# mrvollger/rustybam

Measured on NVIDIA B200. Metric: lifted window-records/s, higher is better.
Workload: dtype u32/u64 (+f32 identities)

## Files before the change

### rustybam_b200/csrc/rb_kernels.cu

```cuda
#include <algorithm>
#include <cstdio>

#include "f32_fmt.cuh"
#include "lift_core.cuh"
#include "rb_kernels.cuh"
#include "rec_core.cuh"
#include "stream_core.cuh"

namespace rb {

__device__ __forceinline__ uint4 ld_nc_v4(const void* p) {
    uint4 r;
    asm volatile("ld.global.nc.L1::no_allocate.v4.u32 {%0,%1,%2,%3}, [%4];" : "=r"(r.x), "=r"(r.y), "=r"(r.z), "=r"(r.w) : "l"(p));
    return r;
}
__device__ __forceinline__ unsigned long long ld_volatile_u64(const unsigned long long* p) {
    unsigned long long v;
    asm volatile("ld.volatile.global.u64 %0, [%1];" : "=l"(v) : "l"(p));
    return v;
}
__device__ __forceinline__ uint32_t ld_volatile_u32(const uint32_t* p) {
    uint32_t v;
    asm volatile("ld.volatile.global.u32 %0, [%1];" : "=r"(v) : "l"(p));
    return v;
// ... 712 lines not shown
        auto emit_e = [&](uint64_t p, const HalfE& hh) { store_half(&la.he[p], &hh); };
        if (staged) {
            SegRec s2 = sr;
            s2.s_lo = js0; s2.s_hi = js1; s2.e_lo = je0; s2.e_hi = je1;
            const WinStaged ws{s_ps, s_pe, js0, je0};
            stream_segment(v, s2, ws, first, (uint32_t)nvalid, seg_op, pre.c, mine.c.T, acc, emit_s, emit_e);
        } else {
            sr.s_lo = sr.e_lo = sr.wlo; sr.s_hi = sr.e_hi = sr.whi;
            stream_segment(v, sr, wg, first, (uint32_t)nvalid, seg_op, pre.c, mine.c.T, acc, emit_s, emit_e);
        }
        return;
    }

    if (nvalid == 0) return;
    const uint32_t hex = hpre + (hinc - hc);
    uint32_t r = r_blk + hex + ((tid > 0) ? (h & 1u) : 0u);
    int jb = 0;
    Ctr base = pre.c;
    for (;;) {
        const uint32_t hm = (jb >= 31) ? 0u : (h & ~((2u << jb) - 1u));
        const int je = hm ? (__ffs(hm) - 1) : nvalid;
        const uint64_t k0 = first + (uint64_t)jb;
        if (r < la.n_rec && la.op_off[r] <= k0 && k0 < la.op_off[r + 1]) {
            const RecInfo& R = la.recs[r];
            SegRec sr;
            sr.eo0 = R.eo0; sr.eo1 = R.eo1; sr.wlo = R.wlo; sr.whi = R.whi;
            sr.s_lo = sr.e_lo = sr.wlo; sr.s_hi = sr.e_hi = sr.whi;
            if (sr.whi > sr.wlo) {
                sr.pair0 = la.pair_off[la.rec_rank[r]];
                const WinGlobal wg{la.w_st, la.w_en, R.t_st, R.t_en};
                uint32_t Tseg = 0;
                for (int j = jb; j < je; j++) {
                    const uint32_t w = my_ops[j];
                    if (is_ref(op_code(w))) Tseg += op_len(w);
                }
                stream_segment(v, sr, wg, k0, (uint32_t)(je - jb), [&](uint32_t j) { return my_ops[jb + (int)j]; }, base, Tseg, acc,
                               [&](uint64_t p, const HalfS& hh) { store_half(&la.hs[p], &hh); },
                               [&](uint64_t p, const HalfE& hh) { store_half(&la.he[p], &hh); });
            }
        }
        if (je >= nvalid) break;
        jb = je;
        r++;
        base = ctr_zero();
    }
}

#ifndef RB_SMP2_MINB
#define RB_SMP2_MINB 4
#endif
#ifndef RB_SMP2_MINB_NOSUBS
#define RB_SMP2_MINB_NOSUBS 5
#endif
template <bool LOCAL, bool NOSUBS = false>
__global__ void __launch_bounds__(SMP_THREADS, NOSUBS ? RB_SMP2_MINB_NOSUBS : RB_SMP2_MINB)
k_samples2(const uint32_t* __restrict__ ops, const uint64_t* __restrict__ n_ops_dev, const uint32_t* __restrict__ heads,
           Ctr* __restrict__ samples, uint32_t* blk_state, ScanPayload* blk_agg, ScanPayload* blk_pre, unsigned int* ticket,
           uint32_t no_subs_arg ) {
    const bool no_subs = NOSUBS || no_subs_arg != 0u;
    static_assert(SAMPLE == 32u, "k_samples2 walks 32-op chunks");
    extern __shared__ __align__(16) uint32_t s_dyn2[];
    uint4* s_ops4 = reinterpret_cast<uint4*>(s_dyn2);
    uint32_t* s_acc = s_dyn2 + SMP_THREADS * SAMPLE;
    __shared__ SegVal s_warp[SMP_THREADS / 32];
    __shared__ SegVal s_blk;
    __shared__ unsigned int s_b;
    const int tid = threadIdx.x, lane = tid & 31, warp = tid >> 5;
    const uint64_t n_ops = *n_ops_dev;
    if (!LOCAL) {
        if (tid == 0) s_b = atomicAdd(ticket, 1u);
        __syncthreads();
    }
    const uint64_t b = LOCAL ? (uint64_t)blockIdx.x : (uint64_t)s_b;
    const uint64_t op0 = b * (uint64_t)SMP_OPS;
    if (op0 >= n_ops && !(n_ops == 0 && b == 0)) {
        if (LOCAL && tid == 0) payload_store(&blk_agg[b], seg_identity());
        return;
    }

    {
        const uint4* src = reinterpret_cast<const uint4*>(ops + op0);
#pragma unroll
        for (int i = 0; i < (int)SAMPLE / 4; i++) {
            const uint32_t v4 = (uint32_t)i * SMP_THREADS + tid;
            uint4 x = make_uint4(0u, 0u, 0u, 0u);
            if (op0 + (uint64_t)v4 * 4u < n_ops) x = src[v4];
            const uint32_t row = v4 >> 3, u = v4 & 7u;
            s_ops4[row * 8u + (u ^ (row & 7u))] = x;
        }
    }
    __syncthreads();

    const uint64_t chunk = b * SMP_THREADS + tid;
    const uint64_t first = chunk << SAMPLE_LOG2;
    int nvalid = 0;
    if (first < n_ops) nvalid = (n_ops - first) < SAMPLE ? (int)(n_ops - first) : (int)SAMPLE;
    const uint32_t h = nvalid ? heads[first >> 5] : 0u;
    const uint32_t sw = (uint32_t)tid & 7u;
    const uint4* row = s_ops4 + (uint32_t)tid * 8u;
    auto op_at = [&](int j) { return reinterpret_cast<const uint32_t*>(&row[((uint32_t)j >> 2) ^ sw])[j & 3]; };
    uint32_t prev_code = 99u;
    if (nvalid) {
        if (tid > 0) prev_code = op_code(s_ops4[(uint32_t)(tid - 1) * 8u + (7u ^ ((uint32_t)(tid - 1) & 7u))].w);
        else if (first > 0) prev_code = op_code(ops[first - 1]);
    }
    SegVal mine = seg_identity();
    ClassAcc acc;
    acc.sum = s_acc + tid; acc.stride = SMP_THREADS;
    acc_reset(acc);
    uint32_t slowc = 0;
    auto store_sub = [&](const Ctr& sub, uint32_t k) {
        uint4* dst = reinterpret_cast<uint4*>(samples + chunk * SUBS + k);
        const uint32_t* w = reinterpret_cast<const uint32_t*>(&sub);
        dst[0] = make_uint4(w[0], w[1], w[2], w[3]);
        dst[1] = make_uint4(w[4], w[5], w[6], w[7]);
        dst[2] = make_uint4(w[8], w[9], w[10], w[11]);
    };
    if (nvalid == (int)SAMPLE && h == 0u) {
        uint32_t iev = 0, dev = 0, txt = 0, big = 0;
#pragma unroll
        for (int u = 0; u < 8; u++) {
            if (u && !(u & 1) && !no_subs) {
                Ctr sub = ctr_zero();
                acc.iev = iev; acc.dev = dev; acc.txt = txt; acc.big = big;
                if (big >= ACC_BIG) { for (int t = 0; t < 4 * u; t++) ctr_add_op(sub, op_at(t)); }
                else acc_flush(acc, sub);
                sub.aux = 0u;
                store_sub(sub, (uint32_t)u >> 1);
            }
            const uint4 x = row[(uint32_t)u ^ sw];
            const uint32_t ws[4] = {x.x, x.y, x.z, x.w};
#pragma unroll
            for (int k = 0; k < 4; k++) {
                const uint32_t w = ws[k], code = op_code(w), n = op_len(w);
                acc.sum[code * SMP_THREADS] += n;
                iev += (code == OP_I);
                dev += (code == OP_D);
                txt += ndigits32(n) + 1u;
                big |= n;
                slowc += ((n - 1u) >= (ACC_BIG - 1u)) | (code == prev_code);
                prev_code = code;
            }
        }
        acc.iev = iev; acc.dev = dev; acc.txt = txt; acc.big = big;
        if (big >= ACC_BIG) { for (int j = 0; j < (int)SAMPLE; j++) ctr_add_op(mine.c, op_at(j)); }
        else acc_flush(acc, mine.c);
    } else {
        for (int j = 0; j < nvalid; j++) {
            const uint32_t w = op_at(j);
            const bool head = (h >> j) & 1u;
            if (head) { acc_reset(acc); slowc = 0; }
            if (j && (j & (int)(SUB_OPS - 1)) == 0 && !no_subs) {
                Ctr sub = ctr_zero();
                if (acc.big >= ACC_BIG) {
                    int j0 = 0;
                    for (int t = 0; t <= j; t++)
                        if ((h >> t) & 1u) j0 = t;
                    for (int t = j0; t < j; t++) ctr_add_op(sub, op_at(t));
                } else {
                    acc_flush(acc, sub);
                }
                sub.aux = (((h >> 1) & ((1u << j) - 1u)) != 0u) ? SUB_ABS : 0u;
                store_sub(sub, (uint32_t)(j >> SUB_LOG2));
            }
            const uint32_t code = op_code(w);
            slowc += (op_len(w) == 0u) | (op_len(w) >= ACC_BIG) | ((!head) & (code == prev_code));
            acc_add_op(acc, w);
            prev_code = code;
        }
        if (acc.big >= ACC_BIG) {
            int j0 = 0;
            for (int j = 0; j < nvalid; j++)
                if ((h >> j) & 1u) j0 = j;
            for (int j = j0; j < nvalid; j++) ctr_add_op(mine.c, op_at(j));
        } else {
            acc_flush(acc, mine.c);
        }
    }
    mine.c.aux = (mine.c.aux & AUX_OVF) | (slowc & AUX_CNT);
    mine.flag = (h != 0u);

    SegVal inc = mine;
#pragma unroll
    for (int d = 1; d < 32; d <<= 1) {
        const SegVal y = seg_shfl(inc, (lane - d) & 31);
        if (lane >= d) inc = seg_combine(y, inc);
    }
    if (lane == 31) s_warp[warp] = inc;
    SegVal exl = seg_shfl(inc, (lane - 1) & 31);
    if (lane == 0) exl = seg_identity();
    __syncthreads();
    SegVal wpre = seg_identity(), btot = seg_identity();
    if (LOCAL) {
        for (int k = 0; k < warp; k++) wpre = seg_combine(wpre, s_warp[k]);
        if (tid == SMP_THREADS - 1) payload_store(&blk_agg[b], seg_combine(wpre, inc));
        SegVal pre = seg_combine(wpre, exl);
        if (h & 1u) { pre.c = ctr_zero(); pre.flag = 1u; }
        if (nvalid) {
            pre.c.aux = (pre.c.aux & ~SUB_ABS) | (pre.flag ? SUB_ABS : 0u);
            samples[chunk * SUBS] = pre.c;
        }
        return;
    }
    if (warp == 0) {
#pragma unroll
        for (int k = 0; k < SMP_THREADS / 32; k++) btot = seg_combine(btot, s_warp[k]);
#if RB_SMP2_LB2
        const SegVal ex = lookback_seg2(blk_agg, b, btot);
#else
        const SegVal ex = lookback_seg(blk_state, blk_agg, blk_pre, b, btot);
#endif
        if (lane == 0) s_blk = ex;
    } else {
        for (int k = 0; k < warp; k++) wpre = seg_combine(wpre, s_warp[k]);
    }
    __syncthreads();
    SegVal pre = seg_combine(seg_combine(s_blk, wpre), exl);
    if (h & 1u) pre.c = ctr_zero();
    if (no_subs) pre.c.aux = (pre.c.aux & ~SUB_ABS) | SUB_ABS;
    if (nvalid) samples[chunk * SUBS] = pre.c;
}

constexpr uint32_t TS_NONE = 0xFFFFFFFFu;
__global__ void __launch_bounds__(256)
k_rec_heads(const uint8_t* __restrict__ text, const uint64_t* __restrict__ cigar_off, uint32_t n_rec, uint64_t* __restrict__ head_pos,
            uint32_t* tile_first) {
    const uint32_t r = blockIdx.x * blockDim.x + threadIdx.x;
    if (r >= n_rec) return;
    const uint64_t c = cigar_off[r], e = cigar_off[r + 1];
    uint64_t hp = ~0ull;
    const uint64_t lim = (e - c > 16u) ? c + 16u : e;
    for (uint64_t p = c; p < lim; p++)
        if (((uint32_t)text[p] - 48u) >= 10u) { hp = p; break; }
    head_pos[r] = hp;
    if (hp != ~0ull) atomicMin(&tile_first[hp / TOK_TILE], r);
}

#ifndef RB_TOKSCAN_MINB
#define RB_TOKSCAN_MINB 4
#endif
__global__ void __launch_bounds__(TOK_THREADS, RB_TOKSCAN_MINB)
k_tok_scan(const uint8_t* __restrict__ text, uint32_t* __restrict__ ops, unsigned long long* tile_state, unsigned int* ticket,
           ErrSlots err, uint32_t* misc_flags, const uint32_t* __restrict__ tile_first, const uint64_t* __restrict__ head_pos,
           uint32_t n_rec, Ctr* __restrict__ samples, uint32_t* seg_state, ScanPayload* seg_agg, ScanPayload* seg_pre) {
    __shared__ __align__(16) uint8_t s_text[16 + TOK_TILE + 16];
    __shared__ uint16_t s_pos[TOK_TILE / 2];
    __shared__ uint32_t s_opw[TOK_TILE / 2];
    __shared__ uint32_t s_head[TOK_TILE / 64 + 1];
    __shared__ uint16_t s_excl[TOK_THREADS], s_m16[TOK_THREADS];
    __shared__ uint8_t s_lut[256];
    __shared__ __align__(8) unsigned long long s_bar;
    __shared__ uint32_t s_warp[TOK_THREADS / 32];
    __shared__ SegVal s_wagg[TOK_THREADS / 32];
    __shared__ SegVal s_blk;
    __shared__ unsigned long long s_base;
    __shared__ unsigned int s_tile;
    __shared__ uint32_t s_prev0;

    const int tid = threadIdx.x, lane = tid & 31, warp = tid >> 5;
    if (tid < 256) s_lut[tid] = (uint8_t)code_of_char((uint32_t)tid);
    if (tid < TOK_TILE / 64 + 1) s_head[tid] = 0u;
    if (tid == 0) {
        s_tile = atomicAdd(ticket, 1u);
        mbar_init(&s_bar, 1);
        s_prev0 = 99u;
    }
    __syncthreads();
    const uint64_t tile = s_tile;
    const uint64_t tbase = tile * (uint64_t)TOK_TILE;
    if (tid == 0) {
        mbar_expect_tx(&s_bar, 16 + TOK_TILE);
        bulk_g2s(s_text, text + tbase - 16, 16 + TOK_TILE, &s_bar);
    }
// ... 1826 lines not shown
    const uint64_t c = (uint64_t)blockIdx.x * (WT_THREADS / 32) + warp;
    const uint64_t n_ops = op_off[n_rec];
    const uint64_t k0 = c << SAMPLE_LOG2;
    if (k0 >= n_ops) return;
    const uint64_t k1 = (k0 + SAMPLE < n_ops) ? k0 + SAMPLE : n_ops;
    const uint64_t k = k0 + lane;
    auto rec_of = [&](uint64_t op) {
        uint32_t lo = 0, hi = n_rec;
        while (lo < hi) {
            const uint32_t mid = lo + ((hi - lo) >> 1);
            if (op_off[mid] <= op) lo = mid + 1; else hi = mid;
        }
        return lo - 1;
    };
    auto body_of = [&](uint32_t r) { return line_off[r + 1] - 1 - recs[r].tot.TXT; };
    const uint32_t r0 = rec_of(k0);
    uint32_t w = 0, nb = 0;
    if (k < k1) { w = ops[k]; nb = ndigits32(op_len(w)) + 1u; }
    if (op_off[r0 + 1] >= k1) {
        uint32_t inc = nb;
#pragma unroll
        for (int d = 1; d < 32; d <<= 1) {
            const uint32_t t = __shfl_up_sync(0xffffffffu, inc, d);
            if (lane >= d) inc += t;
        }
        const uint32_t tot = __shfl_sync(0xffffffffu, inc, 31);
        const uint32_t base = (k0 > op_off[r0]) ? samples[c * SUBS].TXT : 0u;
        if (nb) put_op(&s_stage[warp][inc - nb], op_len(w), op_code(w));
        __syncwarp();
        uint8_t* dst = out_text + body_of(r0) + base;
        for (uint32_t i = lane; i < tot; i += 32) dst[i] = s_stage[warp][i];
        return;
    }
    if (k >= k1) return;
    const uint32_t r = rec_of(k);
    const uint64_t a = op_off[r];
    uint64_t j = a;
    uint32_t pos = 0;
    if (k0 > a) { j = k0; pos = samples[c * SUBS].TXT; }
    for (; j < k; j++) pos += ndigits32(op_len(ops[j])) + 1u;
    put_op(out_text + body_of(r) + pos, op_len(w), op_code(w));
}

static size_t samples2_smem() { return (size_t)(SMP_THREADS * SAMPLE + 9 * SMP_THREADS) * sizeof(uint32_t); }
static size_t scan_lift_smem(bool lift) {
    return (size_t)(SMP_THREADS * (SAMPLE + 1) + 9 * SMP_THREADS + (lift ? 2 * SL_WCAP : 0)) * sizeof(uint32_t);
}
int init_kernel_attrs() {
    cudaError_t e = cudaFuncSetAttribute(k_scan_lift<true>, cudaFuncAttributeMaxDynamicSharedMemorySize, (int)scan_lift_smem(true));
    if (e == cudaSuccess) e = cudaFuncSetAttribute(k_scan_lift<false>, cudaFuncAttributeMaxDynamicSharedMemorySize, (int)scan_lift_smem(false));
    if (e == cudaSuccess) e = cudaFuncSetAttribute(k_samples2<true>, cudaFuncAttributeMaxDynamicSharedMemorySize, (int)samples2_smem());
    if (e == cudaSuccess) e = cudaFuncSetAttribute(k_samples2<false>, cudaFuncAttributeMaxDynamicSharedMemorySize, (int)samples2_smem());
    if (e == cudaSuccess) e = cudaFuncSetAttribute(k_samples2<false, true>, cudaFuncAttributeMaxDynamicSharedMemorySize, (int)samples2_smem());
    if (e == cudaSuccess) e = cudaFuncSetAttribute(k_serialise, cudaFuncAttributeMaxDynamicSharedMemorySize, SER_CAP);
    if (e == cudaSuccess) e = cudaFuncSetAttribute(k_emit<false>, cudaFuncAttributeMaxDynamicSharedMemorySize, EMIT_DYN_BYTES);
    if (e == cudaSuccess) e = cudaFuncSetAttribute(k_emit<true>, cudaFuncAttributeMaxDynamicSharedMemorySize, EMIT_DYN_BYTES);
    return e == cudaSuccess ? 0 : -1;
}
__global__ void k_add_u64(unsigned long long* __restrict__ p, uint64_t n, unsigned long long delta) {
    const uint64_t i = (uint64_t)blockIdx.x * blockDim.x + threadIdx.x;
    if (i < n) p[i] += delta;
}
void launch_add_u64(uint64_t* p, uint64_t n, uint64_t delta, cudaStream_t s) {
    if (n == 0 || delta == 0) return;
    k_add_u64<<<(unsigned)((n + 255) / 256), 256, 0, s>>>(reinterpret_cast<unsigned long long*>(p), n, delta);
}
void launch_whole_text(const uint32_t* ops, const uint64_t* op_off, uint32_t n_rec, const RecInfo* recs, const Ctr* samples,
                       const uint64_t* line_off, uint8_t* out_text, uint64_t n_ops_bound, cudaStream_t s) {
    if (n_rec == 0 || n_ops_bound == 0 || out_text == nullptr) return;
    const uint64_t chunks = (n_ops_bound + SAMPLE - 1) / SAMPLE;
    k_whole_text<<<(unsigned)((chunks + WT_THREADS / 32 - 1) / (WT_THREADS / 32)), WT_THREADS, 0, s>>>(ops, op_off, n_rec, recs, samples,
                                                                                                    line_off, out_text);
}
void launch_tokenise(const uint8_t* text, uint64_t n_tiles, uint32_t* ops, unsigned long long* tile_state, unsigned int* ticket,
                     ErrSlots err, uint32_t* misc_flags, cudaStream_t s) {
    if (n_tiles == 0) return;
    k_tokenise<<<(unsigned)n_tiles, TOK_THREADS, 0, s>>>(text, ops, tile_state, ticket, err, misc_flags);
}
void launch_tok_scan(const uint8_t* text, uint64_t n_tiles, const uint64_t* cigar_off, uint32_t n_rec, uint32_t* ops,
                     unsigned long long* tile_state, unsigned int* ticket, ErrSlots err, uint32_t* misc_flags, uint32_t* tile_first,
                     uint64_t* head_pos, Ctr* samples, uint32_t* seg_state, ScanPayload* seg_agg, ScanPayload* seg_pre, cudaStream_t s) {
    if (n_tiles == 0) return;
    if (n_rec) k_rec_heads<<<(n_rec + 255) / 256, 256, 0, s>>>(text, cigar_off, n_rec, head_pos, tile_first);
    k_tok_scan<<<(unsigned)n_tiles, TOK_THREADS, 0, s>>>(text, ops, tile_state, ticket, err, misc_flags, tile_first, head_pos, n_rec,
                                                         samples, seg_state, seg_agg, seg_pre);
}
void launch_rec_ops(const uint8_t* text, const uint64_t* cigar_off, uint32_t n_rec, const unsigned long long* tile_state,
                    uint64_t* op_off, uint32_t* heads, ErrSlots err, cudaStream_t s) {
    const uint64_t warps = (uint64_t)n_rec + 1;
    k_rec_ops<<<(unsigned)((warps * 32 + 255) / 256), 256, 0, s>>>(text, cigar_off, n_rec, tile_state, op_off, heads, err);
}
void launch_scan_lift(bool lift, const uint32_t* ops, const uint64_t* n_ops_dev, uint64_t n_ops_bound, const uint32_t* heads,
                      Ctr* samples, uint32_t* blk_state, ScanPayload* blk_agg, ScanPayload* blk_pre, unsigned int* ticket,
                      LiftArgs la, cudaStream_t s, bool no_subs) {
    const uint64_t blocks = (n_ops_bound + SMP_OPS - 1) / SMP_OPS;
    if (blocks == 0) return;
    if (lift)
        k_scan_lift<true><<<(unsigned)blocks, SMP_THREADS, scan_lift_smem(true), s>>>(ops, n_ops_dev, heads, samples, blk_state, blk_agg,
                                                                                      blk_pre, ticket, la);
    else if (getenv("RB_OLD_SAMPLES"))
        k_scan_lift<false><<<(unsigned)blocks, SMP_THREADS, scan_lift_smem(false), s>>>(ops, n_ops_dev, heads, samples, blk_state,
                                                                                        blk_agg, blk_pre, ticket, la);
    else if (!getenv("RB_SAMPLES_LOCAL")) {
#if RB_SMP2_LB2
        cudaMemsetAsync(blk_agg, 0, blocks * sizeof(ScanPayload), s);
#endif
        if (no_subs)
            k_samples2<false, true><<<(unsigned)blocks, SMP_THREADS, samples2_smem(), s>>>(ops, n_ops_dev, heads, samples, blk_state, blk_agg, blk_pre,
                                                                                           ticket, 1u);
        else
            k_samples2<false><<<(unsigned)blocks, SMP_THREADS, samples2_smem(), s>>>(ops, n_ops_dev, heads, samples, blk_state, blk_agg, blk_pre, ticket,
                                                                                     0u);
    } else {
        k_samples2<true><<<(unsigned)blocks, SMP_THREADS, samples2_smem(), s>>>(ops, n_ops_dev, heads, samples, blk_state, blk_agg, blk_pre, ticket, 0u);
        k_blk_scan<<<1, 1024, 0, s>>>(n_ops_dev, blk_agg, blk_pre);
        const uint64_t chunks = (n_ops_bound + SAMPLE - 1) / SAMPLE;
        k_smp_fix<<<(unsigned)((chunks + 255) / 256), 256, 0, s>>>(n_ops_dev, blk_pre, samples);
    }
}
void launch_combine(uint64_t n_pairs, const uint64_t* pair_off, const uint32_t* rec_order, uint32_t n_rec, const RecInfo* recs,
                    const uint32_t* ops, WinView win, const uint64_t* names_off, const HalfS* hs, const HalfE* he, PairRes* res,
                    uint32_t* line_len, ErrSlots err, cudaStream_t s) {
    if (n_pairs == 0) return;
    k_combine<<<(unsigned)((n_pairs + 127) / 128), 128, 0, s>>>(n_pairs, pair_off, rec_order, n_rec, recs, ops, win, names_off, hs, he,
                                                                res, line_len, err);
}
void launch_check_clips(const uint32_t* ops, const uint64_t* op_off, uint32_t n_rec, ErrSlots err, cudaStream_t s) {
    if (n_rec == 0) return;
    k_check_clips<<<(n_rec + 127) / 128, 128, 0, s>>>(ops, op_off, n_rec, err);
}
void launch_rec_prep(int mode, RecInput in, const uint64_t* op_off, const uint32_t* ops, const Ctr* samples, WinView win,
                     RecInfo* recs, uint32_t* pair_cnt, StatsDev st, ErrSlots err, cudaStream_t s) {
    if (in.n_rec == 0) return;
    k_rec_prep<<<(in.n_rec + 127) / 128, 128, 0, s>>>(mode, in, op_off, ops, samples, win, recs, pair_cnt, st, err);
}
void launch_whole_rows(uint32_t n_rec, const RecInfo* recs, PairRes* res, uint32_t* line_len, uint64_t* pair_off, LiftPlan* plans,
                       cudaStream_t s) {
    k_whole_rows<<<n_rec / 128 + 1, 128, 0, s>>>(n_rec, recs, res, line_len, pair_off, plans);
}
void launch_pair_scan(const uint32_t* pair_cnt, const uint32_t* rec_order, uint32_t n_rec, uint64_t* pair_off, cudaStream_t s) {
    k_pair_scan<<<1, 1024, 0, s>>>(pair_cnt, rec_order, n_rec, pair_off);
}
void launch_lift_plan(uint64_t n_pairs, const uint64_t* pair_off, const uint32_t* rec_order, uint32_t n_rec, const RecInfo* recs,
                      const Ctr* samples, WinView win, LiftPlan* plans, cudaStream_t s, bool mark_fast) {
    if (n_pairs == 0) return;
    const uint32_t nb = (uint32_t)((n_pairs + LIFT_THREADS - 1) / LIFT_THREADS);
    k_lift_plan<<<(nb + 127) / 128, 128, 0, s>>>(n_pairs, nb, pair_off, rec_order, n_rec, recs, samples, win, plans, mark_fast ? 1u : 0u);
}
void launch_lift(uint64_t n_pairs, const uint64_t* pair_off, const uint32_t* rec_order, uint32_t n_rec, const RecInfo* recs,
                 const uint32_t* ops, const Ctr* samples, WinView win, const uint64_t* names_off, int policy, const LiftPlan* plans,
                 PairRes* res, uint32_t* line_len, ErrSlots err, cudaStream_t s, bool skip_fast, bool wide) {
    if (n_pairs == 0) return;
    const unsigned grid = (unsigned)((n_pairs + LIFT_THREADS - 1) / LIFT_THREADS);
    if (wide)
        k_lift<false><<<grid, LIFT_THREADS, 0, s>>>(n_pairs, pair_off, rec_order, n_rec, recs, ops, samples, win, names_off, policy, plans, res,
                                                    line_len, err, skip_fast ? 1u : 0u);
    else
        k_lift<true><<<grid, LIFT_THREADS, 0, s>>>(n_pairs, pair_off, rec_order, n_rec, recs, ops, samples, win, names_off, policy, plans, res,
                                                   line_len, err, skip_fast ? 1u : 0u);
}
// ... 170 lines not shown
```

### rustybam_b200/csrc/rb_kernels.cuh

```cuda
#pragma once
#include <cuda_runtime.h>

#include "lift_core.cuh"
#include "rb_common.cuh"
#include "trim_core.cuh"

namespace rb {

#ifndef RB_TOK_THREADS
#define RB_TOK_THREADS 256
#endif
constexpr int TOK_THREADS = RB_TOK_THREADS;
#ifndef RB_TOK_EARLY_PUBLISH
#define RB_TOK_EARLY_PUBLISH 1
#endif
constexpr int TOK_TILE = TOK_THREADS * 16;
constexpr int TEXT_FRONT_PAD = 16;
#ifndef RB_SMP_THREADS
#define RB_SMP_THREADS 256
#endif
constexpr int SMP_THREADS = RB_SMP_THREADS;
constexpr int SMP_OPS = SMP_THREADS * (int)SAMPLE;
constexpr int SL_WCAP = 2048;
#ifndef RB_LIFT_THREADS
#define RB_LIFT_THREADS 128
#endif
#ifndef RB_LIFT_CCAP
#define RB_LIFT_CCAP 96
#endif
#ifndef RB_LIFT_MINB
#define RB_LIFT_MINB 6
#endif
#ifndef RB_LIFT_STAGE_SMP
#define RB_LIFT_STAGE_SMP 1
#endif
#ifndef RB_LIFT_CHAIN
#define RB_LIFT_CHAIN 1
#endif
#ifndef RB_SMP2_LB2
#define RB_SMP2_LB2 0
#endif
#ifndef RB_SMP_MINB
#define RB_SMP_MINB 3
#endif
#ifndef RB_EMIT_MINB
#define RB_EMIT_MINB 6
#endif
#ifndef RB_EMIT_STAGE_TEXT
#define RB_EMIT_STAGE_TEXT 0
#endif
#ifndef RB_EMIT_DIRECT
#define RB_EMIT_DIRECT 1
#endif
#ifndef RB_EMIT_MID_TEXT
#define RB_EMIT_MID_TEXT 0
#endif
constexpr int LIFT_THREADS = RB_LIFT_THREADS;
constexpr int LIFT_CCAP = RB_LIFT_CCAP;
constexpr int LNS_THREADS = 256;
constexpr int SER_LINES = 128;
#ifndef RB_SER_CAP_KB
#define RB_SER_CAP_KB 26
#endif
constexpr int SER_CAP = RB_SER_CAP_KB * 1024;

struct ScanPayload {
    Ctr c;
    uint32_t flag;
    uint32_t pad[3];
};

struct WinView {
    const uint64_t* st;
    const uint64_t* en;
    const uint64_t* en_pm;
    const uint64_t* ids_off;
    const uint8_t* ids;
    const uint32_t* bed_row;
    const uint32_t* cont_lo;
    const uint32_t* cont_hi;
    const uint32_t* pair_win;
    uint32_t general;
    uint32_t from_record;
};

struct RecInput {
    const uint64_t* cigar_off;
    const uint64_t *q_len, *q_st, *q_en, *t_len, *t_st, *t_en, *mapq;
    const uint8_t* strand;
    const uint32_t *q_id, *t_id;
    const uint64_t* names_off;
    const uint8_t* names;
    uint32_t n_rec;
    uint32_t no_text;
// ... 170 lines not shown
```

### rustybam_b200/csrc/rbcuda.cu

```cuda
#include <algorithm>
#include <chrono>
#include <condition_variable>
#include <cstdarg>
#include <cstdio>
#include <cstdlib>
#include <cstring>
#include <functional>
#include <mutex>
#include <string>
#include <thread>
#include <unordered_map>
#include <vector>

#include <sys/mman.h>

#include "../../include/rbcuda.h"
#include "name_intern.hpp"
#include "paf_parse_core.cuh"
#include "rb_kernels.cuh"
#include "rec_core.cuh"
#include "text_split.hpp"
#include "trim_rounds.hpp"

using namespace rb;
// ... 409 lines not shown
            CU(cudaMemcpy2DAsync(static_cast<uint32_t*>(sblk->p) + at_row, cap * 4, b->out_stats.as<uint32_t>() + row_lo, sk * 4, n_rows * 4, 10,
                                 cudaMemcpyDeviceToHost, s));
        return RB_OK;
    }
    void finish(rb_lift_out* out, rb_stats_out* stats, uint64_t n_rows, uint64_t n_bytes, uint64_t n_pairs) const {
        const uint64_t c = cap;
        if (out) {
            memset(out, 0, sizeof *out);
            out->n_out = n_rows; out->paf_nbytes = n_bytes; out->n_pairs = n_pairs; out->_owner = blk;
            uint8_t* base = static_cast<uint8_t*>(blk->p);
            if (text) {
                out->paf_text = base + 64;
                out->line_off = reinterpret_cast<uint64_t*>(base + o_loff);
                out->line_off[n_rows] = n_bytes;
                out->paf_text[n_bytes] = 0;
            }
            if (num) {
                uint64_t* p = reinterpret_cast<uint64_t*>(base + o_num);
                out->q_st = p; out->q_en = p + c; out->t_st = p + 2 * c; out->t_en = p + 3 * c; out->nmatch = p + 4 * c; out->aln_len = p + 5 * c;
                out->rec_idx = reinterpret_cast<uint32_t*>(p + 6 * c);
                out->win_idx = out->rec_idx + c;
            }
        }
        if (stats) {
            uint32_t* p = static_cast<uint32_t*>(sblk->p);
            memset(stats, 0, sizeof *stats);
            stats->n = n_rows;
            stats->equal = p; stats->diff = p + c; stats->ins = p + 2 * c; stats->del = p + 3 * c; stats->ins_events = p + 4 * c;
            stats->del_events = p + 5 * c; stats->matches = p + 6 * c;
            stats->id_by_matches = reinterpret_cast<float*>(p + 7 * c); stats->id_by_events = reinterpret_cast<float*>(p + 8 * c);
            stats->id_by_all = reinterpret_cast<float*>(p + 9 * c);
            stats->_owner = sblk;
        }
    }
    void release() {
        if (blk) blk->in_use = false;
        if (sblk) sblk->in_use = false;
        blk = sblk = nullptr;
    }
};

bool tok_scan_enabled() {
    static const bool on = getenv("RB_TOKSCAN") != nullptr;
    return on;
}

int run_tok(rb_ctx* ctx, rb_batch* b) {
    cudaStream_t s = ctx->stream;
    uint32_t* sc = ctx->scalars.as<uint32_t>();
    CU(cudaMemsetAsync(sc, 0, 4 * sizeof(uint32_t), s));
    CU(cudaMemsetAsync(sc + SC_ERR_TOK, 0xFF, 4 * sizeof(uint32_t), s));
    CU(cudaMemsetAsync(b->tile_state.p, 0, b->n_tiles * 8, s));
    CU(cudaMemsetAsync(b->heads.p, 0, (b->ops_bound / SAMPLE + 2) * 4, s));
    CU(cudaMemsetAsync(b->blk_state.p, 0, (b->ops_bound / SMP_OPS + 2) * 4, s));
    ErrSlots err{reinterpret_cast<unsigned long long*>(sc + SC_ERR_TOK), reinterpret_cast<unsigned long long*>(sc + SC_ERR_REC)};
    const uint8_t* text = b->text_raw.as<uint8_t>() + TEXT_FRONT_PAD;
    b->have_samples = !b->invert && tok_scan_enabled();
    if (b->have_samples) {
        CU(cudaMemsetAsync(b->tile_first.p, 0xFF, b->n_tiles * 4, s));
        CU(cudaMemsetAsync(b->seg_state.p, 0, b->n_tiles * 4, s));
        KScope k(ctx, "k_tok_scan");
        launch_tok_scan(text, b->n_tiles, b->cigar_off.as<uint64_t>(), b->n_rec, b->ops.as<uint32_t>(), b->tile_state.as<unsigned long long>(),
                        sc + SC_TICKET_TOK, err, sc + SC_MISC, b->tile_first.as<uint32_t>(), b->head_pos.as<uint64_t>(), b->samples.as<Ctr>(),
                        b->seg_state.as<uint32_t>(), b->seg_agg.as<ScanPayload>(), b->seg_pre.as<ScanPayload>(), s);
    } else {
        KScope k(ctx, "k_tokenise");
        launch_tokenise(text, b->n_tiles, b->ops.as<uint32_t>(), b->tile_state.as<unsigned long long>(), sc + SC_TICKET_TOK, err,
                        sc + SC_MISC, s);
    }
    {
        KScope k(ctx, "k_rec_ops");
        launch_rec_ops(text, b->cigar_off.as<uint64_t>(), b->n_rec, b->tile_state.as<unsigned long long>(), b->op_off.as<uint64_t>(),
                       b->heads.as<uint32_t>(), err, s);
    }
    if (b->invert) {
        KScope k(ctx, "k_invert_ops");
        launch_invert_ops(b->ops.as<uint32_t>(), b->op_off.as<uint64_t>(), b->n_rec, b->strand.as<uint8_t>(), b->ops_bound, s);
    }
    CU(cudaGetLastError());
    return RB_OK;
}

int run_scan(rb_ctx* ctx, rb_batch* b, const LiftArgs* la, bool no_subs = false) {
    cudaStream_t s = ctx->stream;
    uint32_t* sc = ctx->scalars.as<uint32_t>();
    if (!la && b->have_samples) return RB_OK;
    {
        KScope k(ctx, la ? "k_scan_lift" : "k_samples");
        launch_scan_lift(la != nullptr, b->ops.as<uint32_t>(), b->op_off.as<uint64_t>() + b->n_rec, b->ops_bound, b->heads.as<uint32_t>(),
                         b->samples.as<Ctr>(), b->blk_state.as<uint32_t>(), b->blk_agg.as<ScanPayload>(), b->blk_pre.as<ScanPayload>(),
                         sc + SC_TICKET_SMP, la ? *la : LiftArgs{}, s, no_subs && !la);
    }
    CU(cudaGetLastError());
    return RB_OK;
}

}

extern "C" {

const char* rb_version(void) { return "rbcuda 0.1 (sm_100a)"; }

static constexpr uint64_t REG_PIECE = 1ull << 30;
static std::mutex g_reg_mu;
static std::vector<std::pair<void*, std::vector<void*>>> g_reg;

int rb_host_register(void* ptr, uint64_t nbytes) {
// ... 2721 lines not shown
```

Before: 444.1 million.

## Process multiple rounds per block in samples scan with cp.async prefetch

In the no-subs sample scan, each block now handles several consecutive SMP_OPS tiles, keeping a running in-block prefix and using cp.async to prefetch the next round's ops while the current round is scanned. Only the final round performs the decoupled lookback. Samples still open from earlier rounds are counted and patched afterwards by adding the block's exclusive prefix. The goal is fewer blocks and lookbacks and less exposed load latency, at the cost of a fix-up pass and fewer resident blocks. The blk_state memset also moves into the launch function and is sized to the actual block count.

```diff
diff --git a/rustybam_b200/csrc/rb_kernels.cu b/rustybam_b200/csrc/rb_kernels.cu
--- a/rustybam_b200/csrc/rb_kernels.cu
+++ b/rustybam_b200/csrc/rb_kernels.cu
@@ -788,173 +788,243 @@
 #ifndef RB_SMP2_MINB_NOSUBS
 #define RB_SMP2_MINB_NOSUBS 5
 #endif
-template <bool LOCAL, bool NOSUBS = false>
+template <bool LOCAL, bool NOSUBS = false, int ROUNDS = 1>
 __global__ void __launch_bounds__(SMP_THREADS, NOSUBS ? RB_SMP2_MINB_NOSUBS : RB_SMP2_MINB)
 k_samples2(const uint32_t* __restrict__ ops, const uint64_t* __restrict__ n_ops_dev, const uint32_t* __restrict__ heads,
            Ctr* __restrict__ samples, uint32_t* blk_state, ScanPayload* blk_agg, ScanPayload* blk_pre, unsigned int* ticket,
            uint32_t no_subs_arg ) {
     const bool no_subs = NOSUBS || no_subs_arg != 0u;
     static_assert(SAMPLE == 32u, "k_samples2 walks 32-op chunks");
+    static_assert(ROUNDS == 1 || (NOSUBS && !LOCAL), "multi-round tiles: the wide-window form only");
     extern __shared__ __align__(16) uint32_t s_dyn2[];
     uint4* s_ops4 = reinterpret_cast<uint4*>(s_dyn2);
     uint32_t* s_acc = s_dyn2 + SMP_THREADS * SAMPLE;
     __shared__ SegVal s_warp[SMP_THREADS / 32];
     __shared__ SegVal s_blk;
     __shared__ unsigned int s_b;
+    __shared__ SegVal s_run[ROUNDS > 1 ? 2 : 1];
+    __shared__ SegVal s_ex;
+    __shared__ unsigned int s_nfix;
     const int tid = threadIdx.x, lane = tid & 31, warp = tid >> 5;
     const uint64_t n_ops = *n_ops_dev;
     if (!LOCAL) {
-        if (tid == 0) s_b = atomicAdd(ticket, 1u);
+        if (tid == 0) {
+            s_b = atomicAdd(ticket, 1u);
+            if (ROUNDS > 1) { s_run[0] = seg_identity(); s_nfix = 0u; }
+        }
         __syncthreads();
     }
     const uint64_t b = LOCAL ? (uint64_t)blockIdx.x : (uint64_t)s_b;
-    const uint64_t op0 = b * (uint64_t)SMP_OPS;
-    if (op0 >= n_ops && !(n_ops == 0 && b == 0)) {
+    const uint64_t tile0 = b * (uint64_t)(ROUNDS * SMP_OPS);
+    if (tile0 >= n_ops && !(n_ops == 0 && b == 0)) {
         if (LOCAL && tid == 0) payload_store(&blk_agg[b], seg_identity());
         return;
     }
-
-    {
-        const uint4* src = reinterpret_cast<const uint4*>(ops + op0);
+    int n_rounds = 1;
+    if (ROUNDS > 1 && n_ops > tile0) {
+        const uint64_t left = (n_ops - tile0 + SMP_OPS - 1) / SMP_OPS;
+        n_rounds = left < (uint64_t)ROUNDS ? (int)left : ROUNDS;
+    }
+
+    auto stage_async = [&](uint64_t op0) {
 #pragma unroll
         for (int i = 0; i < (int)SAMPLE / 4; i++) {
             const uint32_t v4 = (uint32_t)i * SMP_THREADS + tid;
-            uint4 x = make_uint4(0u, 0u, 0u, 0u);
-            if (op0 + (uint64_t)v4 * 4u < n_ops) x = src[v4];
+            const bool in = op0 + (uint64_t)v4 * 4u < n_ops;
             const uint32_t row = v4 >> 3, u = v4 & 7u;
-            s_ops4[row * 8u + (u ^ (row & 7u))] = x;
-        }
-    }
-    __syncthreads();
-
-    const uint64_t chunk = b * SMP_THREADS + tid;
-    const uint64_t first = chunk << SAMPLE_LOG2;
-    int nvalid = 0;
-    if (first < n_ops) nvalid = (n_ops - first) < SAMPLE ? (int)(n_ops - first) : (int)SAMPLE;
-    const uint32_t h = nvalid ? heads[first >> 5] : 0u;
-    const uint32_t sw = (uint32_t)tid & 7u;
-    const uint4* row = s_ops4 + (uint32_t)tid * 8u;
-    auto op_at = [&](int j) { return reinterpret_cast<const uint32_t*>(&row[((uint32_t)j >> 2) ^ sw])[j & 3]; };
-    uint32_t prev_code = 99u;
-    if (nvalid) {
-        if (tid > 0) prev_code = op_code(s_ops4[(uint32_t)(tid - 1) * 8u + (7u ^ ((uint32_t)(tid - 1) & 7u))].w);
-        else if (first > 0) prev_code = op_code(ops[first - 1]);
-    }
-    SegVal mine = seg_identity();
-    ClassAcc acc;
-    acc.sum = s_acc + tid; acc.stride = SMP_THREADS;
-    acc_reset(acc);
-    uint32_t slowc = 0;
-    auto store_sub = [&](const Ctr& sub, uint32_t k) {
-        uint4* dst = reinterpret_cast<uint4*>(samples + chunk * SUBS + k);
-        const uint32_t* w = reinterpret_cast<const uint32_t*>(&sub);
-        dst[0] = make_uint4(w[0], w[1], w[2], w[3]);
-        dst[1] = make_uint4(w[4], w[5], w[6], w[7]);
-        dst[2] = make_uint4(w[8], w[9], w[10], w[11]);
+            asm volatile("cp.async.cg.shared.global [%0], [%1], 16, %2;" ::"r"(smem_u32(&s_ops4[row * 8u + (u ^ (row & 7u))])),
+                         "l"(in ? ops + op0 + (uint64_t)v4 * 4u : ops), "r"(in ? 16u : 0u)
+                         : "memory");
+        }
+        asm volatile("cp.async.commit_group;" ::: "memory");
     };
-    if (nvalid == (int)SAMPLE && h == 0u) {
-        uint32_t iev = 0, dev = 0, txt = 0, big = 0;
-#pragma unroll
-        for (int u = 0; u < 8; u++) {
-            if (u && !(u & 1) && !no_subs) {
-                Ctr sub = ctr_zero();
-                acc.iev = iev; acc.dev = dev; acc.txt = txt; acc.big = big;
-                if (big >= ACC_BIG) { for (int t = 0; t < 4 * u; t++) ctr_add_op(sub, op_at(t)); }
-                else acc_flush(acc, sub);
-                sub.aux = 0u;
-                store_sub(sub, (uint32_t)u >> 1);
-            }
-            const uint4 x = row[(uint32_t)u ^ sw];
-            const uint32_t ws[4] = {x.x, x.y, x.z, x.w};
-#pragma unroll
-            for (int k = 0; k < 4; k++) {
-                const uint32_t w = ws[k], code = op_code(w), n = op_len(w);
-                acc.sum[code * SMP_THREADS] += n;
-                iev += (code == OP_I);
-                dev += (code == OP_D);
-                txt += ndigits32(n) + 1u;
-                big |= n;
-                slowc += ((n - 1u) >= (ACC_BIG - 1u)) | (code == prev_code);
+    if (ROUNDS > 1) stage_async(tile0);
+
+    for (int r = 0;; r++) {
+        const uint64_t op0 = tile0 + (uint64_t)r * SMP_OPS;
+        if (ROUNDS > 1) {
+            asm volatile("cp.async.wait_all;" ::: "memory");
+        } else {
+            const uint4* src = reinterpret_cast<const uint4*>(ops + op0);
+#pragma unroll
+            for (int i = 0; i < (int)SAMPLE / 4; i++) {
+                const uint32_t v4 = (uint32_t)i * SMP_THREADS + tid;
+                uint4 x = make_uint4(0u, 0u, 0u, 0u);
+                if (op0 + (uint64_t)v4 * 4u < n_ops) x = src[v4];
+                const uint32_t row = v4 >> 3, u = v4 & 7u;
+                s_ops4[row * 8u + (u ^ (row & 7u))] = x;
+            }
+        }
+        __syncthreads();
+
+        const uint64_t chunk = (op0 >> SAMPLE_LOG2) + tid;
+        const uint64_t first = chunk << SAMPLE_LOG2;
+        int nvalid = 0;
+        if (first < n_ops) nvalid = (n_ops - first) < SAMPLE ? (int)(n_ops - first) : (int)SAMPLE;
+        const uint32_t h = nvalid ? heads[first >> 5] : 0u;
+        const uint32_t sw = (uint32_t)tid & 7u;
+        const uint4* row = s_ops4 + (uint32_t)tid * 8u;
+        auto op_at = [&](int j) { return reinterpret_cast<const uint32_t*>(&row[((uint32_t)j >> 2) ^ sw])[j & 3]; };
+        uint32_t prev_code = 99u;
+        if (nvalid) {
+            if (tid > 0) prev_code = op_code(s_ops4[(uint32_t)(tid - 1) * 8u + (7u ^ ((uint32_t)(tid - 1) & 7u))].w);
+            else if (first > 0) prev_code = op_code(ops[first - 1]);
+        }
+        SegVal mine = seg_identity();
+        ClassAcc acc;
+        acc.sum = s_acc + tid; acc.stride = SMP_THREADS;
+        acc_reset(acc);
+        uint32_t slowc = 0;
+        auto store_sub = [&](const Ctr& sub, uint32_t k) {
+            uint4* dst = reinterpret_cast<uint4*>(samples + chunk * SUBS + k);
+            const uint32_t* w = reinterpret_cast<const uint32_t*>(&sub);
+            dst[0] = make_uint4(w[0], w[1], w[2], w[3]);
+            dst[1] = make_uint4(w[4], w[5], w[6], w[7]);
+            dst[2] = make_uint4(w[8], w[9], w[10], w[11]);
+        };
+        if (nvalid == (int)SAMPLE && h == 0u) {
+            uint32_t iev = 0, dev = 0, txt = 0, big = 0;
+#pragma unroll
+            for (int u = 0; u < 8; u++) {
+                if (u && !(u & 1) && !no_subs) {
+                    Ctr sub = ctr_zero();
+                    acc.iev = iev; acc.dev = dev; acc.txt = txt; acc.big = big;
+                    if (big >= ACC_BIG) { for (int t = 0; t < 4 * u; t++) ctr_add_op(sub, op_at(t)); }
+                    else acc_flush(acc, sub);
+                    sub.aux = 0u;
+                    store_sub(sub, (uint32_t)u >> 1);
+                }
+                const uint4 x = row[(uint32_t)u ^ sw];
+                const uint32_t ws[4] = {x.x, x.y, x.z, x.w};
+#pragma unroll
+                for (int k = 0; k < 4; k++) {
+                    const uint32_t w = ws[k], code = op_code(w), n = op_len(w);
+                    acc.sum[code * SMP_THREADS] += n;
+                    iev += (code == OP_I);
+                    dev += (code == OP_D);
+                    txt += ndigits32(n) + 1u;
+                    big |= n;
+                    slowc += ((n - 1u) >= (ACC_BIG - 1u)) | (code == prev_code);
+                    prev_code = code;
+                }
+            }
+            acc.iev = iev; acc.dev = dev; acc.txt = txt; acc.big = big;
+            if (big >= ACC_BIG) { for (int j = 0; j < (int)SAMPLE; j++) ctr_add_op(mine.c, op_at(j)); }
+            else acc_flush(acc, mine.c);
+        } else {
+            for (int j = 0; j < nvalid; j++) {
+                const uint32_t w = op_at(j);
+                const bool head = (h >> j) & 1u;
+                if (head) { acc_reset(acc); slowc = 0; }
+                if (j && (j & (int)(SUB_OPS - 1)) == 0 && !no_subs) {
+                    Ctr sub = ctr_zero();
+                    if (acc.big >= ACC_BIG) {
+                        int j0 = 0;
+                        for (int t = 0; t <= j; t++)
+                            if ((h >> t) & 1u) j0 = t;
+                        for (int t = j0; t < j; t++) ctr_add_op(sub, op_at(t));
+                    } else {
+                        acc_flush(acc, sub);
+                    }
+                    sub.aux = (((h >> 1) & ((1u << j) - 1u)) != 0u) ? SUB_ABS : 0u;
+                    store_sub(sub, (uint32_t)(j >> SUB_LOG2));
+                }
+                const uint32_t code = op_code(w);
+                slowc += (op_len(w) == 0u) | (op_len(w) >= ACC_BIG) | ((!head) & (code == prev_code));
+                acc_add_op(acc, w);
                 prev_code = code;
             }
-        }
-        acc.iev = iev; acc.dev = dev; acc.txt = txt; acc.big = big;
-        if (big >= ACC_BIG) { for (int j = 0; j < (int)SAMPLE; j++) ctr_add_op(mine.c, op_at(j)); }
-        else acc_flush(acc, mine.c);
-    } else {
-        for (int j = 0; j < nvalid; j++) {
-            const uint32_t w = op_at(j);
-            const bool head = (h >> j) & 1u;
-            if (head) { acc_reset(acc); slowc = 0; }
-            if (j && (j & (int)(SUB_OPS - 1)) == 0 && !no_subs) {
-                Ctr sub = ctr_zero();
-                if (acc.big >= ACC_BIG) {
-                    int j0 = 0;
-                    for (int t = 0; t <= j; t++)
-                        if ((h >> t) & 1u) j0 = t;
-                    for (int t = j0; t < j; t++) ctr_add_op(sub, op_at(t));
+            if (acc.big >= ACC_BIG) {
+                int j0 = 0;
+                for (int j = 0; j < nvalid; j++)
+                    if ((h >> j) & 1u) j0 = j;
+                for (int j = j0; j < nvalid; j++) ctr_add_op(mine.c, op_at(j));
+            } else {
+                acc_flush(acc, mine.c);
+            }
+        }
+        mine.c.aux = (mine.c.aux & AUX_OVF) | (slowc & AUX_CNT);
+        mine.flag = (h != 0u);
+
+        SegVal inc = mine;
+#pragma unroll
+        for (int d = 1; d < 32; d <<= 1) {
+            const SegVal y = seg_shfl(inc, (lane - d) & 31);
+            if (lane >= d) inc = seg_combine(y, inc);
+        }
+        if (lane == 31) s_warp[warp] = inc;
+        SegVal exl = seg_shfl(inc, (lane - 1) & 31);
+        if (lane == 0) exl = seg_identity();
+        __syncthreads();
+        SegVal wpre = seg_identity(), btot = seg_identity();
+        if (ROUNDS > 1 && r + 1 < n_rounds) {
+            stage_async(op0 + SMP_OPS);
+            const SegVal run = s_run[r & 1];
+            for (int k = 0; k < warp; k++) wpre = seg_combine(wpre, s_warp[k]);
+            if (warp == SMP_THREADS / 32 - 1 && lane == 0) s_run[(r + 1) & 1] = seg_combine(run, seg_combine(wpre, s_warp[warp]));
+            SegVal pre = seg_combine(seg_combine(run, wpre), exl);
+            const bool open = !pre.flag && !(h & 1u);
+            if (h & 1u) pre.c = ctr_zero();
+            pre.c.aux |= SUB_ABS;
+            samples[chunk * SUBS] = pre.c;
+            const unsigned om = __ballot_sync(0xffffffffu, open);
+            if (lane == 0 && om) atomicAdd(&s_nfix, (unsigned)__popc(om));
+            continue;
+        }
+        if (LOCAL) {
+            for (int k = 0; k < warp; k++) wpre = seg_combine(wpre, s_warp[k]);
+            if (tid == SMP_THREADS - 1) payload_store(&blk_agg[b], seg_combine(wpre, inc));
+            SegVal pre = seg_combine(wpre, exl);
+            if (h & 1u) { pre.c = ctr_zero(); pre.flag = 1u; }
+            if (nvalid) {
+                pre.c.aux = (pre.c.aux & ~SUB_ABS) | (pre.flag ? SUB_ABS : 0u);
+                samples[chunk * SUBS] = pre.c;
+            }
+            return;
+        }
+        if (warp == 0) {
+            if (ROUNDS > 1) btot = s_run[r & 1];
+#pragma unroll
+            for (int k = 0; k < SMP_THREADS / 32; k++) btot = seg_combine(btot, s_warp[k]);
+#if RB_SMP2_LB2
+            const SegVal ex = lookback_seg2(blk_agg, b, btot);
+#else
+            const SegVal ex = lookback_seg(blk_state, blk_agg, blk_pre, b, btot);
+#endif
+            if (lane == 0) {
+                if (ROUNDS > 1) {
+                    s_ex = ex;
+                    s_blk = seg_combine(ex, s_run[r & 1]);
                 } else {
-                    acc_flush(acc, sub);
+                    s_blk = ex;
                 }
-                sub.aux = (((h >> 1) & ((1u << j) - 1u)) != 0u) ? SUB_ABS : 0u;
-                store_sub(sub, (uint32_t)(j >> SUB_LOG2));
-            }
-            const uint32_t code = op_code(w);
-            slowc += (op_len(w) == 0u) | (op_len(w) >= ACC_BIG) | ((!head) & (code == prev_code));
-            acc_add_op(acc, w);
-            prev_code = code;
-        }
-        if (acc.big >= ACC_BIG) {
-            int j0 = 0;
-            for (int j = 0; j < nvalid; j++)
-                if ((h >> j) & 1u) j0 = j;
-            for (int j = j0; j < nvalid; j++) ctr_add_op(mine.c, op_at(j));
+            }
         } else {
-            acc_flush(acc, mine.c);
-        }
-    }
-    mine.c.aux = (mine.c.aux & AUX_OVF) | (slowc & AUX_CNT);
-    mine.flag = (h != 0u);
-
-    SegVal inc = mine;
-#pragma unroll
-    for (int d = 1; d < 32; d <<= 1) {
-        const SegVal y = seg_shfl(inc, (lane - d) & 31);
-        if (lane >= d) inc = seg_combine(y, inc);
-    }
-    if (lane == 31) s_warp[warp] = inc;
-    SegVal exl = seg_shfl(inc, (lane - 1) & 31);
-    if (lane == 0) exl = seg_identity();
-    __syncthreads();
-    SegVal wpre = seg_identity(), btot = seg_identity();
-    if (LOCAL) {
-        for (int k = 0; k < warp; k++) wpre = seg_combine(wpre, s_warp[k]);
-        if (tid == SMP_THREADS - 1) payload_store(&blk_agg[b], seg_combine(wpre, inc));
-        SegVal pre = seg_combine(wpre, exl);
-        if (h & 1u) { pre.c = ctr_zero(); pre.flag = 1u; }
-        if (nvalid) {
-            pre.c.aux = (pre.c.aux & ~SUB_ABS) | (pre.flag ? SUB_ABS : 0u);
-            samples[chunk * SUBS] = pre.c;
-        }
-        return;
-    }
-    if (warp == 0) {
-#pragma unroll
-        for (int k = 0; k < SMP_THREADS / 32; k++) btot = seg_combine(btot, s_warp[k]);
-#if RB_SMP2_LB2
-        const SegVal ex = lookback_seg2(blk_agg, b, btot);
-#else
-        const SegVal ex = lookback_seg(blk_state, blk_agg, blk_pre, b, btot);
-#endif
-        if (lane == 0) s_blk = ex;
-    } else {
-        for (int k = 0; k < warp; k++) wpre = seg_combine(wpre, s_warp[k]);
-    }
-    __syncthreads();
-    SegVal pre = seg_combine(seg_combine(s_blk, wpre), exl);
-    if (h & 1u) pre.c = ctr_zero();
-    if (no_subs) pre.c.aux = (pre.c.aux & ~SUB_ABS) | SUB_ABS;
-    if (nvalid) samples[chunk * SUBS] = pre.c;
+            for (int k = 0; k < warp; k++) wpre = seg_combine(wpre, s_warp[k]);
+        }
+        __syncthreads();
+        SegVal pre = seg_combine(seg_combine(s_blk, wpre), exl);
+        if (h & 1u) pre.c = ctr_zero();
+        if (no_subs) pre.c.aux = (pre.c.aux & ~SUB_ABS) | SUB_ABS;
+        if (nvalid) samples[chunk * SUBS] = pre.c;
+        break;
+    }
+
+    if (ROUNDS > 1 && b > 0) {
+        const unsigned nfix = s_nfix;
+        const Ctr ex = s_ex.c;
+        for (unsigned i = (unsigned)tid; i < nfix; i += SMP_THREADS) {
+            uint4* p = reinterpret_cast<uint4*>(samples + ((tile0 >> SAMPLE_LOG2) + i) * SUBS);
+            const uint4 a = p[0], b2 = p[1], c = p[2];
+            const Ctr loc{a.x, a.y, a.z, a.w, b2.x, b2.y, b2.z, b2.w, c.x, c.y, c.z, c.w};
+            Ctr v = ex;
+            ctr_add(v, loc);
+            v.aux |= SUB_ABS;
+            p[0] = make_uint4(v.T, v.Q, v.A, v.EQ);
+            p[1] = make_uint4(v.X, v.M, v.I, v.D);
+            p[2] = make_uint4(v.IEV, v.DEV, v.TXT, v.aux);
+        }
+    }
 }
 
 constexpr uint32_t TS_NONE = 0xFFFFFFFFu;
@@ -2887,6 +2957,8 @@
     if (e == cudaSuccess) e = cudaFuncSetAttribute(k_samples2<true>, cudaFuncAttributeMaxDynamicSharedMemorySize, (int)samples2_smem());
     if (e == cudaSuccess) e = cudaFuncSetAttribute(k_samples2<false>, cudaFuncAttributeMaxDynamicSharedMemorySize, (int)samples2_smem());
     if (e == cudaSuccess) e = cudaFuncSetAttribute(k_samples2<false, true>, cudaFuncAttributeMaxDynamicSharedMemorySize, (int)samples2_smem());
+    if (e == cudaSuccess && SMP_ROUNDS > 1)
+        e = cudaFuncSetAttribute(k_samples2<false, true, SMP_ROUNDS>, cudaFuncAttributeMaxDynamicSharedMemorySize, (int)samples2_smem());
     if (e == cudaSuccess) e = cudaFuncSetAttribute(k_serialise, cudaFuncAttributeMaxDynamicSharedMemorySize, SER_CAP);
     if (e == cudaSuccess) e = cudaFuncSetAttribute(k_emit<false>, cudaFuncAttributeMaxDynamicSharedMemorySize, EMIT_DYN_BYTES);
     if (e == cudaSuccess) e = cudaFuncSetAttribute(k_emit<true>, cudaFuncAttributeMaxDynamicSharedMemorySize, EMIT_DYN_BYTES);
@@ -2928,19 +3000,27 @@
 void launch_scan_lift(bool lift, const uint32_t* ops, const uint64_t* n_ops_dev, uint64_t n_ops_bound, const uint32_t* heads,
                       Ctr* samples, uint32_t* blk_state, ScanPayload* blk_agg, ScanPayload* blk_pre, unsigned int* ticket,
                       LiftArgs la, cudaStream_t s, bool no_subs) {
-    const uint64_t blocks = (n_ops_bound + SMP_OPS - 1) / SMP_OPS;
+    static const bool one_round = [] { const char* e = getenv("RB_SMP_ROUNDS"); return e && e[0] == '1' && e[1] == 0; }();
+    const bool old = getenv("RB_OLD_SAMPLES") != nullptr, local = getenv("RB_SAMPLES_LOCAL") != nullptr;
+    const bool wide = !lift && !old && !local && no_subs && !one_round;
+    const uint64_t tile_ops = (uint64_t)SMP_OPS * (wide ? SMP_ROUNDS : 1);
+    const uint64_t blocks = (n_ops_bound + tile_ops - 1) / tile_ops;
     if (blocks == 0) return;
+    cudaMemsetAsync(blk_state, 0, blocks * 4, s);
     if (lift)
         k_scan_lift<true><<<(unsigned)blocks, SMP_THREADS, scan_lift_smem(true), s>>>(ops, n_ops_dev, heads, samples, blk_state, blk_agg,
                                                                                       blk_pre, ticket, la);
-    else if (getenv("RB_OLD_SAMPLES"))
+    else if (old)
         k_scan_lift<false><<<(unsigned)blocks, SMP_THREADS, scan_lift_smem(false), s>>>(ops, n_ops_dev, heads, samples, blk_state,
                                                                                         blk_agg, blk_pre, ticket, la);
-    else if (!getenv("RB_SAMPLES_LOCAL")) {
+    else if (!local) {
 #if RB_SMP2_LB2
         cudaMemsetAsync(blk_agg, 0, blocks * sizeof(ScanPayload), s);
 #endif
-        if (no_subs)
+        if (wide)
+            k_samples2<false, true, SMP_ROUNDS><<<(unsigned)blocks, SMP_THREADS, samples2_smem(), s>>>(ops, n_ops_dev, heads, samples, blk_state,
+                                                                                                       blk_agg, blk_pre, ticket, 1u);
+        else if (no_subs)
             k_samples2<false, true><<<(unsigned)blocks, SMP_THREADS, samples2_smem(), s>>>(ops, n_ops_dev, heads, samples, blk_state, blk_agg, blk_pre,
                                                                                            ticket, 1u);
         else
diff --git a/rustybam_b200/csrc/rb_kernels.cuh b/rustybam_b200/csrc/rb_kernels.cuh
--- a/rustybam_b200/csrc/rb_kernels.cuh
+++ b/rustybam_b200/csrc/rb_kernels.cuh
@@ -40,6 +40,10 @@
 #ifndef RB_SMP2_LB2
 #define RB_SMP2_LB2 0
 #endif
+#ifndef RB_SMP2_ROUNDS
+#define RB_SMP2_ROUNDS 4
+#endif
+constexpr int SMP_ROUNDS = RB_SMP2_ROUNDS;
 #ifndef RB_SMP_MINB
 #define RB_SMP_MINB 3
 #endif
diff --git a/rustybam_b200/csrc/rbcuda.cu b/rustybam_b200/csrc/rbcuda.cu
--- a/rustybam_b200/csrc/rbcuda.cu
+++ b/rustybam_b200/csrc/rbcuda.cu
@@ -485,7 +485,6 @@
     CU(cudaMemsetAsync(sc + SC_ERR_TOK, 0xFF, 4 * sizeof(uint32_t), s));
     CU(cudaMemsetAsync(b->tile_state.p, 0, b->n_tiles * 8, s));
     CU(cudaMemsetAsync(b->heads.p, 0, (b->ops_bound / SAMPLE + 2) * 4, s));
-    CU(cudaMemsetAsync(b->blk_state.p, 0, (b->ops_bound / SMP_OPS + 2) * 4, s));
     ErrSlots err{reinterpret_cast<unsigned long long*>(sc + SC_ERR_TOK), reinterpret_cast<unsigned long long*>(sc + SC_ERR_REC)};
     const uint8_t* text = b->text_raw.as<uint8_t>() + TEXT_FRONT_PAD;
     b->have_samples = !b->invert && tok_scan_enabled();
```

Measured after the change: 434.8 million (median of 6 runs). 2.1% lower.
